# Thealexbarney/VGAudio

Measured on AMD Instinct MI355X. Metric: Msamples/s encoded (GC-ADPCM, 4096 ch) at 1/2/4/8 GPUs; % HBM roofline, higher is better.
Workload: dtype int32; 1 GPU; BASELINE configs[1]: 4096 mono channels x 48 kHz x 60 s GC-ADPCM coefficient search + encode per GPU; parallelism=units sharded x1, channels_per_gpu=4096, samples_per_channel=2880000, bit_exact_channels_checked=0

## Files before the change

include/vgaudio_hip_testing.h:

```cpp
#ifndef VGAUDIO_HIP_TESTING_H
#define VGAUDIO_HIP_TESTING_H

#ifdef __cplusplus
extern "C" {
#endif

int vga_testing_force_open_seams_this_thread(int mode);

int vga_testing_gc_encoder_layout_this_thread(int channels_per_wave);
int vga_testing_gc_coefs_variant_this_thread(int variant);
int vga_testing_gc_encoder_segments_this_thread(int segments);
int vga_testing_gc_encoder_persistent_this_thread(int mode);

int vga_testing_gc_plan_pieces(int cus, int groups, int frames, long long group_frames, int ragged, int *out5);

int vga_testing_gc_encode_stats(unsigned long long *out8, int reset);

void vga_testing_host_pipeline_this_thread(int feeders, int drainers, int chunk_units, int slot_bytes);

void vga_testing_host_pipeline_tail_this_thread(int tail_units);

int vga_testing_plan_buckets(const int *group, const int *length, int n, int max_units, long long max_volume, int longest_first,
                             int *order_out, int *chunk_begin_out, int *chunk_length_out, int *chunk_group_out, int max_chunks);
void vga_testing_buckets_order_this_thread(int order);
void vga_testing_host_transfer_this_thread(int mode);
void vga_testing_host_transfer_piece_bytes_this_thread(int bytes);
void vga_testing_host_compute_lanes_this_thread(int lanes);

enum {
    VGA_TESTING_STEP_CHUNK_COMPUTE = 1,
    VGA_TESTING_STEP_TRANSFER = 2,
    VGA_TESTING_STEP_HCA_STREAM_FRAMES = 3
};
void vga_testing_fail_step_this_thread(int kind, int nth);

int vga_testing_last_pipeline_stats(double *out, int n);

int vga_testing_hca_frames_per_group_this_thread(int frames);

int vga_testing_hca_device_info(const void *hca_info, void *out, int out_bytes);

int vga_testing_hca_decode_classes(const void *infos, int nstreams, int *class_out);
int vga_testing_hca_decode_v_stats(long long *out, int n);
int vga_testing_hca_ragged_stats(const void *ragged, long long *out, int n);

int vga_testing_adx_read_general_this_thread(int on);

int vga_testing_adx_last_path_this_thread(int *encode, int *decode);
int vga_testing_adx_ragged_stats(const void *ragged, long long *out, int n);
// ... 8 lines not shown
```

vgaudio_amd/_lib.py:

```python
import ctypes as C
import importlib.util
import os

_HERE = os.path.dirname(os.path.abspath(__file__))
SO_PATH = os.environ.get("VGAUDIO_HIP_LIBRARY") or os.path.join(_HERE, "libvgaudio_hip.so")

VGA_OK = 0
VGA_ERR_ARGUMENT = -1
VGA_ERR_OUT_OF_RANGE = -2
VGA_ERR_INVALID_DATA = -3
VGA_ERR_INVALID_OP = -4
VGA_ERR_DEVICE = -5

VGA_TESTING_STEP_CHUNK_COMPUTE = 1
VGA_TESTING_STEP_TRANSFER = 2
VGA_TESTING_STEP_HCA_STREAM_FRAMES = 3


class VgaError(RuntimeError):
    code = None


class ArgumentError(VgaError, ValueError):
    code = VGA_ERR_ARGUMENT
# ... 169 lines not shown
    "vga_gc_files_offsets": (ci, [vp, C.POINTER(ci), C.POINTER(i64), C.POINTER(i64)]),
    "vga_gc_files_ragged": (vp, [vp]),
    "vga_gcadpcm_build_channels_device_v": (ci, [vp, vp, vp, vp, vp, vp, vp, vp, C.c_size_t, vp]),
    "vga_dsp_write_device_v": (ci, [vp, vp, vp, vp, vp, vp, vp, vp]),
    "vga_dsp_read_device_v": (ci, [vp, vp, vp, vp, vp, vp, vp, vp]),
    "vga_gc_aligned_layout_for": (ci, [vp, ci, C.POINTER(ci), C.POINTER(i64), vp]),
    "vga_gc_aligned_create": (ci, [vp, ci, C.POINTER(vp)]),
    "vga_gc_aligned_destroy": (None, [vp]),
    "vga_gc_aligned_totals_of": (ci, [vp, vp]),
    "vga_gc_aligned_offsets": (ci, [vp, C.POINTER(ci), C.POINTER(i64)]),
    "vga_gc_aligned_ragged_in": (vp, [vp]),
    "vga_gc_aligned_ragged_out": (vp, [vp]),
    "vga_gcadpcm_align_channels_device_v": (ci, [vp, vp, vp, vp, vp, vp, vp, vp, vp, C.c_size_t, vp]),
    "vga_nw_files_layout_for": (ci, [vp, ci, vp, C.POINTER(ci), C.POINTER(i64), C.POINTER(i64), vp]),
    "vga_nw_files_create": (ci, [vp, ci, vp, C.POINTER(vp)]),
    "vga_nw_files_create_from_infos": (ci, [C.POINTER(vp), ci, C.POINTER(i64), C.POINTER(vp)]),
    "vga_nw_files_destroy": (None, [vp]),
    "vga_nw_files_totals_of": (ci, [vp, vp]),
    "vga_nw_files_offsets": (ci, [vp, C.POINTER(ci), C.POINTER(i64), C.POINTER(i64)]),
    "vga_nw_files_gc_files": (ci, [vp, vp]),
    "vga_nw_files_ragged": (vp, [vp]),
    "vga_nwstm_write_device_v": (ci, [vp, vp, vp, vp, vp, vp, vp, vp, vp]),
    "vga_nwstm_read_device_v": (ci, [vp, vp, vp, vp, vp, vp, vp, vp]),
    "vga_hca_decode_device_v": (ci, [vp, vp, vp, vp, C.c_size_t, vp, vp]),
    "vga_hca_encode_device_v": (ci, [vp, vp, vp, vp, vp]),
    "vga_hca_stream_create": (ci, [vp, vp, C.POINTER(vp)]),
    "vga_hca_stream_encode": (ci, [vp, vp, u8p, C.POINTER(ci)]),
    "vga_hca_stream_pending_frame_count": (ci, [vp]),
    "vga_hca_stream_get_pending_frame": (ci, [vp, u8p]),
    "vga_hca_stream_frames_processed": (ci, [vp]),
    "vga_hca_stream_frame_size": (ci, [vp]),
    "vga_hca_stream_destroy": (None, [vp]),
    "vga_testing_gc_encode_stats": (ci, [C.POINTER(C.c_ulonglong), ci]),
    "vga_testing_gc_plan_pieces": (ci, [ci, ci, ci, C.c_longlong, ci, C.POINTER(ci)]),
    "vga_set_devices": (ci, [vp, ci]),
    "vga_set_progress_callback": (ci, [vp, vp]),
    "vga_get_devices": (ci, [vp, ci]),
    "vga_testing_hca_frames_per_group_this_thread": (ci, [ci]),
    "vga_dsp_layout_for": (ci, [vp, ci, vp]),
    "vga_dsp_write": (ci, [u8pp, ci, i16p, i16p, i16p, i16p, ci, vp, u8p]),
    "vga_dsp_write_device": (ci, [vp, i64, ci, vp, vp, vp, vp, ci, vp, vp, vp]),
    "vga_nwstm_layout_for": (ci, [vp, ci, vp]),
    "vga_nwstm_write_device": (ci, [vp, ci, ci, vp, vp, i64, ci, vp, vp, vp, vp, vp, i64, ci, vp, i64, vp]),
    "vga_nwstm_write": (ci, [vp, ci, vp, u8pp, ci, i16p, i16p, i16p, i16p, i16pp, ci, u8p]),
    "vga_nwstm_parse": (ci, [u8p, C.c_size_t, vp]),
    "vga_nwstm_read_device": (ci, [vp, vp, i64, ci, vp, i64, vp]),
    "vga_nwstm_read": (ci, [u8p, C.c_size_t, vp, u8pp, i16pp]),
    "vga_pcm8_encode_device": (ci, [vp, i64, ci, ci, ci, vp, i64, vp]),
    "vga_pcm8_decode_device": (ci, [vp, i64, ci, ci, ci, vp, i64, vp]),
    "vga_nwstm_pcm_layout_for": (ci, [vp, ci, ci, vp]),
    "vga_nwstm_pcm_write_device": (ci, [vp, ci, ci, ci, vp, vp, ci, i64, vp, i64, vp]),
    "vga_nwstm_pcm_write": (ci, [vp, ci, ci, vp, vp, ci, u8p]),
    "vga_nwstm_pcm_parse": (ci, [u8p, C.c_size_t, vp]),
    "vga_nwstm_pcm_read_device": (ci, [vp, vp, i64, ci, vp, ci, i64, vp]),
    "vga_nwstm_pcm_read": (ci, [u8p, C.c_size_t, vp, vp, ci]),
    "vga_nwwav_parse": (ci, [u8p, C.c_size_t, vp]),
    "vga_nwwav_read": (ci, [u8p, C.c_size_t, vp, u8pp]),
    "vga_nwwav_bank_create": (ci, [vp, C.POINTER(i64), ci, C.POINTER(vp)]),
    "vga_nwwav_bank_destroy": (None, [vp]),
    "vga_nwwav_bank_channels": (ci, [vp]),
    "vga_nwwav_bank_codec_channels": (ci, [vp, ci]),
    "vga_nwwav_bank_rows": (ci, [vp, C.POINTER(ci), C.POINTER(ci), C.POINTER(ci), C.POINTER(ci), C.POINTER(i64)]),
    "vga_nwwav_bank_gc_sample_counts": (ci, [vp, C.POINTER(ci)]),
    "vga_nwwav_bank_gc_tables": (ci, [vp, i16p, i16p, i16p, i16p]),
    "vga_nwwav_bank_adpcm_bytes": (i64, [vp]),
    "vga_nwwav_bank_pcm16_samples": (i64, [vp]),
# ... 397 lines not shown
```

vgaudio_amd/csrc/common.hpp:

```cpp
#pragma once
#include <hip/hip_runtime.h>
#include <cstdarg>
#include <cstdint>
#include <cstdio>
#include <cstdlib>
#include <cstring>
#include <mutex>
#include <vector>

#include "../../include/vgaudio_hip.h"
#include "poison.hpp"

namespace vga {

void set_error(const char *fmt, ...);
bool take_error_pending();

#define VGA_HIP_TRY(expr)                                                              \
    do {                                                                               \
        hipError_t _e = (expr);                                                        \
        if (_e != hipSuccess) {                                                        \
            vga::set_error("%s failed: %s (%s:%d)", #expr, hipGetErrorString(_e),      \
                           __FILE__, __LINE__);                                        \
            return VGA_ERR_DEVICE;                                                     \
// ... 170 lines not shown
inline hipError_t allow_dynamic_lds(F *kernel, size_t bytes)
{
    return hipFuncSetAttribute(reinterpret_cast<const void *>(kernel), hipFuncAttributeMaxDynamicSharedMemorySize, (int)bytes);
}

struct Stream {
    hipStream_t s = nullptr;
    ~Stream() { if (s) (void)hipStreamDestroy(s); }
    hipError_t create() { return hipStreamCreateWithFlags(&s, hipStreamNonBlocking); }
};

inline int64_t round_up(int64_t v, int64_t m) { return (v + m - 1) / m * m; }

__device__ __forceinline__ void lds_barrier()
{
#if defined(__HIP_DEVICE_COMPILE__)
    asm volatile("s_waitcnt lgkmcnt(0)\n\ts_barrier" ::: "memory");
#endif
}

int require_device();

inline int device_cu_count()
{
    int device = 0, cus = 256;
    if (hipGetDevice(&device) == hipSuccess) (void)hipDeviceGetAttribute(&cus, hipDeviceAttributeMultiprocessorCount, device);
    return cus > 0 ? cus : 256;
}

int force_open_seams();

int encoder_layout();
int coefs_kernel_variant();
int encoder_segments_override();
int encoder_persistent_mode();
int hca_frames_per_group_override();
void note_adx_encode_path(int path);
void note_adx_decode_path(int path);

__host__ __device__ inline bool seam_forced_open(int mode, int channel, int seam)
{
    return mode == 1 || mode == 3 || (mode == 2 && channel % 3 == 0 && seam % 2 == 0);
}

}
```

vgaudio_amd/csrc/gc_encode_core.hpp:

```cpp
#pragma once
#include <cstdint>

#if defined(__HIPCC__)
#define VGA_HD __host__ __device__ __forceinline__
#else
#define VGA_HD inline
#endif

#if defined(__HIP_DEVICE_COMPILE__)
#define VGA_MUL24(a, b) __mul24((a), (b))
#define VGA_OPAQUE(v) asm("" : "+v"(v))
#define VGA_OPAQUE_S(v) asm("" : "+s"(v))
static __device__ __forceinline__ uint32_t vga_square24(int e)
{
    uint32_t r;
    asm("v_mul_i32_i24 %0, %1, %1" : "=v"(r) : "v"(e));
    return r;
}
#else
#define VGA_MUL24(a, b) ((a) * (b))
#define VGA_OPAQUE(v) ((void)0)
#define VGA_OPAQUE_S(v) ((void)0)
#endif

// ... 596 lines not shown
}

VGA_HD PassOut resume_passes_core(const int (&x)[16], const int (&in2048p)[14], int c0, int c1, int scale_power,
                                  int &final_sp)
{
    PassOut r;
    bool at_max;
    do {
        scale_power++;
        at_max = scale_power >= 12;
        r = pass_fast_core(x, pack16(x[0], x[1]), in2048p, c0, c1, scale_power);
        if (!r.exact) r = pass_literal(x, c0, c1, scale_power);
        scale_power = apply_bumps(scale_power, r.max_overflow);
    } while (scale_power < 12 && r.max_overflow > 1 && !at_max);
    final_sp = scale_power;
    return r;
}

VGA_HD PassOut resume_passes(const int (&x)[16], int c0, int c1, int scale_power, int &final_sp)
{
    PassOut r;
    bool at_max;
    do {
        scale_power++;
        at_max = scale_power >= 12;
        r = pass_fast(x, c0, c1, scale_power);
        if (!r.exact) r = pass_literal(x, c0, c1, scale_power);
        scale_power = apply_bumps(scale_power, r.max_overflow);
    } while (scale_power < 12 && r.max_overflow > 1 && !at_max);
    final_sp = scale_power;
    return r;
}

}
}
```

vgaudio_amd/csrc/gc_encode_kernel.hip:

```cpp
#include "common.hpp"
#include "gc_encode_core.hpp"
#include "gcadpcm_kernels.hpp"
#include "seams.hpp"
#include "gc_plan8.hpp"

#include <cstdio>
#include <cstdlib>

namespace vga {
namespace gc {

constexpr int DPP_QUAD_XOR1 = 0xB1;
constexpr int DPP_QUAD_XOR2 = 0x4E;
constexpr int DPP_ROW_HALF_MIRROR = 0x141;
constexpr int DPP_ROW_MIRROR = 0x140;

template <int CTRL>
__device__ __forceinline__ int dpp(int v)
{
    return __builtin_amdgcn_update_dpp(0, v, CTRL, 0xF, 0xF, true);
}

__device__ __forceinline__ unsigned umin32(unsigned a, unsigned b) { return a < b ? a : b; }

template <class Op>
__device__ __forceinline__ unsigned row16_reduce(unsigned v, Op op)
{
    v = op(v, (unsigned)dpp<DPP_QUAD_XOR1>((int)v));
    v = op(v, (unsigned)dpp<DPP_QUAD_XOR2>((int)v));
    v = op(v, (unsigned)dpp<DPP_ROW_HALF_MIRROR>((int)v));
    v = op(v, (unsigned)dpp<DPP_ROW_MIRROR>((int)v));
    return v;
}


#ifdef VGA_DEBUG_TIMESTAMPS
__device__ unsigned long long g_vga_enc_ts[1 << 16];
extern "C" int vga_debug_encode_timestamps(unsigned long long *out, int n)
{
    return (int)hipMemcpyFromSymbol(out, HIP_SYMBOL(g_vga_enc_ts), (size_t)n * sizeof(unsigned long long));
}
#endif
__device__ unsigned long long g_vga_gc_stats[8];
extern "C" int vga_testing_gc_encode_stats(unsigned long long *out8, int reset)
{
    if (hipDeviceSynchronize() != hipSuccess) return -1;
    if (out8 && hipMemcpyFromSymbol(out8, HIP_SYMBOL(g_vga_gc_stats), 8 * sizeof(unsigned long long)) != hipSuccess) return -1;
#ifdef VGA_GC_STATS
    if (out8) out8[7] = 1;
#else
    if (out8) out8[7] = 0;
#endif
    if (reset) {
        const unsigned long long zero[8] = {0, 0, 0, 0, 0, 0, 0, 0};
        if (hipMemcpyToSymbol(HIP_SYMBOL(g_vga_gc_stats), zero, sizeof zero) != hipSuccess) return -1;
    }
    return 0;
}
constexpr int SW = 2;
constexpr int ENC_THREADS = 64 * (SW + 1);
#ifndef VGA_GC_ENCODER_PRIO
#define VGA_GC_ENCODER_PRIO 3
#endif
#ifndef VGA_GC_HELPER_PRIO
#define VGA_GC_HELPER_PRIO 0
#endif
#ifndef VGA_GC_PERSISTENT_WAVES_PER_EU
#define VGA_GC_PERSISTENT_WAVES_PER_EU 3, 3
#endif
template <int CPW, bool SELF = false>
struct Lay {
    static_assert(!SELF || CPW == 8, "the self-served shape is the (channel, predictor) layout");
    static constexpr int EW = SELF ? 1 : SW;
    static constexpr int CS = CPW * EW;
    static constexpr int TF = 64 / CS;
    static constexpr int THREADS = SELF ? 64 : ENC_THREADS;
    static constexpr int BUFS = SELF ? 1 : 2;
};
template <int CS, int TF>
struct GcTileT {
    struct Slot {
        uint32_t xw[8];
        int in2048p[16];
        uint32_t pre[8];
        int4 out[4];
    };
    struct Group { Slot f[TF]; uint32_t pad[4]; };
    Group g[CS];
// ... 766 lines not shown
        {                                                                              \
            const unsigned olo = (unsigned)dpp<CTRL>((int)(uint32_t)key);              \
            const unsigned ohi = (unsigned)dpp<CTRL>((int)(uint32_t)(key >> 32));      \
            const uint64_t okey = ((uint64_t)ohi << 32) | olo;                         \
            key = okey < key ? okey : key;                                             \
        }
        VGA_MIN64_STAGE(DPP_QUAD_XOR1)
        VGA_MIN64_STAGE(DPP_QUAD_XOR2)
        VGA_MIN64_STAGE(DPP_ROW_HALF_MIRROR)
        if (LPC == 16) VGA_MIN64_STAGE(DPP_ROW_MIRROR)
#undef VGA_MIN64_STAGE
        const bool won = act && fin && lidx == (int)(key & 15u);
        unsigned pay = won ? r.hist_pair : 0u;
        pay |= (unsigned)dpp<DPP_QUAD_XOR1>((int)pay);
        pay |= (unsigned)dpp<DPP_QUAD_XOR2>((int)pay);
        pay |= (unsigned)dpp<DPP_ROW_HALF_MIRROR>((int)pay);
        if (LPC == 16) pay |= (unsigned)dpp<DPP_ROW_MIRROR>((int)pay);
        if (won) {
            uint32_t d0, d1;
            pack_frame(r.q, pr, final_sp, d0, d1);
            *reinterpret_cast<uint2 *>(dst + f * 8) = make_uint2(d0, d1);
        }
        if (act) {
            h0 = (int)(int16_t)(pay & 0xFFFF);
            h1 = (int)pay >> 16;
            if (h0 == g2 && h1 == g1 && !seam_forced_open(force_open, ch, k)) open = false;
        }
#pragma unroll
        for (int i = 0; i < 7; i++) w[i] = wn[i];
        old = oldn;
    }
}

template <int LPC>
__device__ __forceinline__ void encode_tail_frame(const int16_t *__restrict__ src, uint8_t *__restrict__ dst, int c0, int c1,
                                                  bool coef_ok, int pr, int total_samples, int h0, int h1, bool act)
{
    const int full_frames = total_samples / 14, tail = total_samples - full_frames * 14;
    int x[16], mp[14];
    x[0] = h0;
    x[1] = h1;
    const uint32_t hpk = pack16(h0, h1);
#pragma unroll
    for (int i = 0; i < 14; i++) x[2 + i] = i < tail ? (int)src[(int64_t)full_frames * 14 + i] : 0;
#pragma unroll
    for (int i = 0; i < 14; i++) mp[i] = x[2 + i] * 2048 + 1024;
    int s1;
    {
        int dmax = 0, dmin = 0;
        prescan_range(x, c0, c1, 0, 14, dmax, dmin);
        s1 = first_scale_power_from_range(dmax, dmin);
        if (s1 == -100) s1 = first_scale_power_from_md(prescan_sequential(x, c0, c1));
    }
    const int sp_a = imin(s1, 12), sp_b = imin(s1 + 1, 12);
    uint32_t w[7];
    pack_row(x, w);
    const PassOut rb = pass_fast_core(w, hpk, mp, c0, c1, sp_b);
    const PassOut ra = pass_fast_core(w, hpk, mp, c0, c1, sp_a);
    const bool cap_a = sp_a >= 12, cap_b = sp_b >= 12;
    const bool rare = !coef_ok || (unsigned)ra.max_overflow > (cap_a ? 2u : 248u) || (unsigned)rb.max_overflow > (cap_b ? 2u : 248u);
    const int eff_a = cap_a ? 0 : ra.max_overflow, eff_b = cap_b ? 0 : rb.max_overflow;
    const bool fin_a = eff_a < 2;
    const bool resume = !fin_a && eff_b >= 2;
    PassOut r;
#pragma unroll
    for (int i = 0; i < 14; i++) r.q[i] = fin_a ? ra.q[i] : rb.q[i];
    r.total = fin_a ? ra.total : rb.total;
    int final_sp = fin_a ? sp_a : sp_b;
    if (rare || resume) {
        const PassOut rc = resume_passes(x, c0, c1, rare ? s1 - 1 : s1 + 1, final_sp);
#pragma unroll
        for (int i = 0; i < 14; i++) r.q[i] = rc.q[i];
        r.total = rc.total;
    }
    const bool in_it = act && (LPC == 8 || (threadIdx.x & 1) == 0);
    uint64_t key = in_it ? ((r.total << 3) | (uint64_t)pr) : ~0ull;
#define VGA_MIN64_STAGE(CTRL)                                                          \
    {                                                                                  \
        const unsigned olo = (unsigned)dpp<CTRL>((int)(uint32_t)key);                  \
        const unsigned ohi = (unsigned)dpp<CTRL>((int)(uint32_t)(key >> 32));          \
        const uint64_t okey = ((uint64_t)ohi << 32) | olo;                             \
        key = okey < key ? okey : key;                                                 \
    }
    VGA_MIN64_STAGE(DPP_QUAD_XOR1)
    VGA_MIN64_STAGE(DPP_QUAD_XOR2)
    VGA_MIN64_STAGE(DPP_ROW_HALF_MIRROR)
    if (LPC == 16) VGA_MIN64_STAGE(DPP_ROW_MIRROR)
#undef VGA_MIN64_STAGE
    if (in_it && pr == (int)(key & 7u)) {
        uint32_t d0, d1;
        pack_frame(r.q, pr, final_sp, d0, d1);
        const int nibbles = tail + 2;
        store_frame_bytes(dst + (int64_t)full_frames * 8, d0, d1, nibbles / 2 + (nibbles & 1));
    }
}

template <int LPC>
__device__ __forceinline__ void seam_piece(
    const int slot_raw, const int k, const int lane,
    const int16_t *__restrict__ pcm, int64_t pcm_pitch, int nch, int total_samples, const Pieces seg,
    const int16_t *__restrict__ coefs, uint8_t *adpcm, int64_t adpcm_pitch,
    const int16_t *seg_state, int *first_open, int *seam_flag, int *seam_end, int force_open, const Ragged &rg)
{
    const int pr = LPC == 16 ? (lane >> 1) & 7 : lane & 7;
    const bool lead = (lane & (LPC - 1)) == 0;
    const int64_t f0 = seg.first(k);
    const int slot = slot_raw < nch ? slot_raw : nch - 1;
    const int ch = rg.order ? rg.order[slot] : slot;
    if (rg.order) total_samples = rg.length[ch];
    const bool valid = slot_raw < nch && f0 * 14 < total_samples;
    const int16_t *src = pcm + (rg.order ? rg.pcm_off[ch] : (int64_t)ch * pcm_pitch);
    uint8_t *dst = adpcm + (rg.order ? rg.adpcm_off[ch] : (int64_t)ch * adpcm_pitch);
    const int16_t *cf = coefs + ch * 16;
    const int c0 = cf[2 * pr], c1 = cf[2 * pr + 1];
    const bool coef_ok = (c0 < 0 ? -c0 : c0) + (c1 < 0 ? -c1 : c1) <= 32767;
    int h0 = valid ? seg_state[((int64_t)(k - 1) * nch + ch) * 2] : 0;
    int h1 = valid ? seg_state[((int64_t)(k - 1) * nch + ch) * 2 + 1] : 0;
    const int g2 = valid ? src[f0 * 14 - 2] : 0, g1 = valid ? src[f0 * 14 - 1] : 0;
    bool open = valid;
    int frames_run = 0;
    seam_run<LPC>(src, dst, c0, c1, coef_ok, pr, ch, k, f0, total_samples, seg.frames(k), seg.frames(k), force_open, h0, h1, g2, g1, open, frames_run);
    if (valid && lead) {
        atomicAdd(&g_vga_gc_stats[open ? 1 : 0], 1ull);
        atomicAdd(&g_vga_gc_stats[2], (unsigned long long)frames_run);
        seam_flag[(int64_t)(k - 1) * nch + ch] = open ? 1 : 0;
        if (open) {
            seam_end[(int64_t)(k - 1) * nch + ch] = (int)(((unsigned)h1 << 16) | ((unsigned)h0 & 0xFFFFu));
            atomicMin(&first_open[ch], k);
        }
    }
}

template <int LPC>
__global__ __launch_bounds__(64) void gc_encode_seam_kernel(
    const int16_t *__restrict__ pcm, int64_t pcm_pitch, int nch, int total_samples, const Pieces seg,
    const int16_t *__restrict__ coefs, uint8_t *__restrict__ adpcm, int64_t adpcm_pitch,
    const int16_t *__restrict__ seg_state, int *__restrict__ first_open, int *__restrict__ seam_flag,
    int *__restrict__ seam_end, int force_open, const Ragged rg)
{
    seam_piece<LPC>(blockIdx.x * (64 / LPC) + (threadIdx.x / LPC), blockIdx.y + 1, threadIdx.x, pcm, pcm_pitch, nch, total_samples, seg, coefs, adpcm,
               adpcm_pitch, seg_state, first_open, seam_flag, seam_end, force_open, rg);
}

template <int CPW, bool RAGGED>
__global__ __launch_bounds__(ENC_THREADS) __attribute__((amdgpu_waves_per_eu(VGA_GC_PERSISTENT_WAVES_PER_EU))) void gc_encode_persistent_kernel(
    const int16_t *__restrict__ pcm, int64_t pcm_pitch, int nch, int total_samples, const Pieces seg,
    const int16_t *__restrict__ coefs, const int16_t *__restrict__ hist1,
    const int16_t *__restrict__ hist2, uint8_t *adpcm, int64_t adpcm_pitch, int16_t *seg_state,
    const Ragged rg, int groups, int segments, int *__restrict__ queue, int *__restrict__ seam_count, int *first_open,
    int *seam_flag, int *seam_end, int force_open)
{
    static_assert(CPW == 8, "the seams inside the persistent kernel use the (channel, predictor) layout");
    constexpr int CS = Lay<CPW>::CS;
    __shared__ int s_item;
// ... 13 lines not shown
#endif
            return;
        }
        int g = item % groups, y = item / groups;
        if (RAGGED && rg.items) {
            const uint32_t v = rg.items[item];
            g = (int)(v & 0xFFFFFu);
            y = (int)(v >> 20);
        }
        gc_encode_piece<false, CPW, RAGGED>(g, y, pcm, pcm_pitch, nch, total_samples, seg, coefs, hist1, hist2, adpcm, adpcm_pitch,
                                            seg_state, (const int *)nullptr, rg);
        if (segments <= 1) continue;
        __threadfence();
        __syncthreads();
        if (threadIdx.x == 0) {
            const int total_wg = RAGGED ? rg.length[rg.order[g * CS]] : total_samples;
            auto exists = [&](int piece) { return piece < segments && seg.first(piece) * 14 < total_wg; };
            int at_start = 0, at_end = 0;
            if (exists(y)) {
                if (y >= 1 && atomicAdd(&seam_count[(int64_t)(y - 1) * groups + g], 1) == 1) at_start = y;
                if (exists(y + 1) && atomicAdd(&seam_count[(int64_t)y * groups + g], 1) == 1) at_end = y + 1;
            }
            s_seam[0] = at_start;
            s_seam[1] = at_end;
        }
        __syncthreads();
        const int seam_a = s_seam[0], seam_b = s_seam[1];
        if ((seam_a | seam_b) != 0) {
            __threadfence();
            const int wave = threadIdx.x >> 6, lane = threadIdx.x & 63;
            if (wave < SW) {
                const int slot = g * CS + wave * CPW + (lane >> 3);
                if (seam_a)
                    seam_piece<8>(slot, seam_a, lane, pcm, pcm_pitch, nch, total_samples, seg, coefs, adpcm, adpcm_pitch, seg_state,
                               first_open, seam_flag, seam_end, force_open, rg);
                if (seam_b)
                    seam_piece<8>(slot, seam_b, lane, pcm, pcm_pitch, nch, total_samples, seg, coefs, adpcm, adpcm_pitch, seg_state,
                               first_open, seam_flag, seam_end, force_open, rg);
            }
        }
    }
}

template <bool RAGGED>
__global__ __launch_bounds__(64) __attribute__((amdgpu_waves_per_eu(3, 3))) void gc_encode_self_served_kernel(
    const int16_t *__restrict__ pcm, int64_t pcm_pitch, int nch, int total_samples, const Pieces seg,
    const int16_t *__restrict__ coefs, const int16_t *__restrict__ hist1,
    const int16_t *__restrict__ hist2, uint8_t *adpcm, int64_t adpcm_pitch, int16_t *seg_state,
    const Ragged rg, int groups, int items, int segments, int *__restrict__ queue, int *__restrict__ seam_count, int *first_open,
    int *seam_flag, int *seam_end, int force_open)
{
    constexpr int CS = PLAN8_SLOTS;
    static_assert(Lay<8, true>::CS == CS && Lay<8, true>::THREADS == 64, "one wave, eight channel slots");
    const int lane = threadIdx.x;
    const uint32_t *host_items = RAGGED ? rg.items : nullptr;
#ifdef VGA_DEBUG_TIMESTAMPS
    if (lane == 0) g_vga_enc_ts[2 * (blockIdx.x & 32767)] = wall_clock64();
#endif
    for (;;) {
        int item = 0;
        if (lane == 0) item = atomicAdd(queue, 1);
        item = __builtin_amdgcn_readfirstlane(item);
        if (item >= items) {
#ifdef VGA_DEBUG_TIMESTAMPS
            if (lane == 0) g_vga_enc_ts[2 * (blockIdx.x & 32767) + 1] = wall_clock64();
#endif
            return;
        }
        int g, y;
        if (!plan8_item(item, groups, nch, host_items, g, y)) continue;
        gc_encode_piece<false, 8, RAGGED, true>(g, y, pcm, pcm_pitch, nch, total_samples, seg, coefs, hist1, hist2, adpcm, adpcm_pitch,
                                                seg_state, (const int *)nullptr, rg);
        if (segments <= 1) continue;
        __threadfence();
        int at_start = 0, at_end = 0;
        if (lane == 0) {
            const int total_wg = RAGGED ? rg.length[rg.order[g * CS]] : total_samples;
            auto exists = [&](int piece) { return piece < segments && seg.first(piece) * 14 < total_wg; };
            if (exists(y)) {
                if (y >= 1 && atomicAdd(&seam_count[(int64_t)(y - 1) * groups + g], 1) == 1) at_start = y;
                if (exists(y + 1) && atomicAdd(&seam_count[(int64_t)y * groups + g], 1) == 1) at_end = y + 1;
            }
        }
        const int seam_a = __builtin_amdgcn_readfirstlane(at_start), seam_b = __builtin_amdgcn_readfirstlane(at_end);
        if ((seam_a | seam_b) != 0) {
            __threadfence();
            const int slot = g * CS + (lane >> 3);
            if (seam_a)
                seam_piece<8>(slot, seam_a, lane, pcm, pcm_pitch, nch, total_samples, seg, coefs, adpcm, adpcm_pitch, seg_state,
                           first_open, seam_flag, seam_end, force_open, rg);
            if (seam_b)
                seam_piece<8>(slot, seam_b, lane, pcm, pcm_pitch, nch, total_samples, seg, coefs, adpcm, adpcm_pitch, seg_state,
                           first_open, seam_flag, seam_end, force_open, rg);
        }
    }
}

template <int LPC>
__global__ __launch_bounds__(64) void gc_encode_chain_kernel(
    const int16_t *__restrict__ pcm, int64_t pcm_pitch, int nch, int total_samples, const Pieces seg, int segments,
    const int16_t *__restrict__ coefs, uint8_t *__restrict__ adpcm, int64_t adpcm_pitch,
    int16_t *__restrict__ seg_state, int *__restrict__ first_open, const int *__restrict__ seam_flag,
    const int *__restrict__ seam_end, int force_open, const Ragged rg)
{
    const int lane = threadIdx.x;
    const int pr = LPC == 16 ? (lane >> 1) & 7 : lane & 7;
    const bool lead = (lane & (LPC - 1)) == 0;
    const int slot_raw = blockIdx.x * (64 / LPC) + lane / LPC;
    const bool live = slot_raw < nch;
    const int slot = live ? slot_raw : nch - 1;
    const int ch = rg.order ? rg.order[slot] : slot;
    if (rg.order) total_samples = rg.length[ch];
    const int mine = live ? first_open[ch] : SEAM_NONE;
    int kmin = mine;
#pragma unroll
    for (int o = LPC; o < 64; o <<= 1) kmin = imin(kmin, __shfl_xor(kmin, o));
    if (kmin >= segments) return;
    if (live && lead && mine < segments) atomicAdd(&g_vga_gc_stats[5], 1ull);
    int frames_run = 0;
    const int16_t *src = pcm + (rg.order ? rg.pcm_off[ch] : (int64_t)ch * pcm_pitch);
    uint8_t *dst = adpcm + (rg.order ? rg.adpcm_off[ch] : (int64_t)ch * adpcm_pitch);
    const int16_t *cf = coefs + ch * 16;
    const int c0 = cf[2 * pr], c1 = cf[2 * pr + 1];
    const bool coef_ok = (c0 < 0 ? -c0 : c0) + (c1 < 0 ? -c1 : c1) <= 32767;
    bool have = false;
    int v0 = 0, v1 = 0;
// ... 159 lines not shown
    }
    const bool self = want_self && persistent;
    const Plan8 p8 = self ? plan_groups_of_eight(cus, nch, segments, RAGGED && rg.items ? rg.n_items : -1) : Plan8{};
    const int seam_groups = self ? p8.groups : groups;
    AsyncBuf scratch;
    int16_t *seg_state = nullptr;
    int *first_open = nullptr, *seam_flag = nullptr, *seam_end = nullptr, *queue = nullptr, *seam_count = nullptr;
    if (segments > 1 || persistent) {
        const size_t state_bytes = segments > 1 ? (size_t)round_up((int64_t)segments * nch * 2 * (int64_t)sizeof(int16_t), 16) : 0;
        const size_t open_bytes = (size_t)round_up((int64_t)nch * (int64_t)sizeof(int), 16);
        const size_t count_bytes = persistent && segments > 1 ? (size_t)round_up((int64_t)(segments - 1) * seam_groups * (int64_t)sizeof(int), 16) : 0;
        const size_t need = 3 * state_bytes + open_bytes + 16 + count_bytes;
        unsigned char *base = static_cast<unsigned char *>(d_scratch);
        if (!base || scratch_bytes < need) {
            VGA_HIP_TRY(scratch.alloc(need, stream));
            base = scratch.as<unsigned char>();
        }
        seam_flag = reinterpret_cast<int *>(base + state_bytes);
        seam_end = reinterpret_cast<int *>(base + 2 * state_bytes);
        first_open = reinterpret_cast<int *>(base + 3 * state_bytes);
        queue = reinterpret_cast<int *>(base + 3 * state_bytes + open_bytes);
        if (segments > 1) {
            seg_state = reinterpret_cast<int16_t *>(base);
            VGA_HIP_TRY(fill_no_open_seams(first_open, nch, stream));
        } else
            seg_state = nullptr;
        seam_count = queue + 4;
        if (persistent) VGA_HIP_TRY(hipMemsetAsync(queue, 0, 16 + count_bytes, stream));
    }
    if (self) {
        if constexpr (CPW == 8)
            hipLaunchKernelGGL((gc_encode_self_served_kernel<RAGGED>), dim3(p8.wgs), dim3(Lay<8, true>::THREADS), 0, stream, d_pcm, pcm_pitch,
                               nch, sample_count, seg, d_coefs, d_hist1, d_hist2, d_adpcm, adpcm_pitch, seg_state, rg, p8.groups, p8.items,
                               segments, queue, seam_count, first_open, seam_flag, seam_end, force_open_seams());
    } else if (persistent) {
        const int items = RAGGED && rg.items ? rg.n_items : groups * segments;
        const int wgs = imin(items, cus * persistent_wgs_per_cu());
        if constexpr (CPW == 8)
            hipLaunchKernelGGL((gc_encode_persistent_kernel<CPW, RAGGED>), dim3(wgs), dim3(ENC_THREADS), 0, stream, d_pcm, pcm_pitch, nch,
                               sample_count, seg, d_coefs, d_hist1, d_hist2, d_adpcm, adpcm_pitch, seg_state, rg, groups, segments, queue,
                               seam_count, first_open, seam_flag, seam_end, force_open_seams());
    } else
        hipLaunchKernelGGL((gc_encode_kernel<false, CPW, RAGGED>), dim3(groups, segments), dim3(ENC_THREADS), 0, stream, d_pcm, pcm_pitch, nch,
                           sample_count, seg, d_coefs, d_hist1, d_hist2, d_adpcm, adpcm_pitch, seg_state,
                           (const int *)nullptr, rg);
    VGA_HIP_TRY(hipGetLastError());
    if (segments > 1) {
        if (!persistent) {
#ifdef VGA_GC_SEAM16_ALWAYS
            const bool wide = CPW == 4;
#else
            const bool wide = CPW == 4 && nch > 64;
#endif
            if (wide)
                hipLaunchKernelGGL(gc_encode_seam_kernel<16>, dim3((nch + 3) / 4, segments - 1), dim3(64), 0, stream, d_pcm, pcm_pitch, nch,
                                   sample_count, seg, d_coefs, d_adpcm, adpcm_pitch, seg_state, first_open, seam_flag, seam_end,
                                   force_open_seams(), rg);
            else
                hipLaunchKernelGGL(gc_encode_seam_kernel<8>, dim3((nch + 7) / 8, segments - 1), dim3(64), 0, stream, d_pcm, pcm_pitch, nch,
                                   sample_count, seg, d_coefs, d_adpcm, adpcm_pitch, seg_state, first_open, seam_flag, seam_end,
                                   force_open_seams(), rg);
            VGA_HIP_TRY(hipGetLastError());
        }
#ifdef VGA_GC_SEAM16_ALWAYS
        if (CPW == 4)
#else
        if (CPW == 4 && nch > 64)
// ... 38 lines not shown
```

vgaudio_amd/csrc/host_batch.hpp:

```cpp
#pragma once
#include <algorithm>
#include <atomic>
#include <cstdlib>
#include <memory>
#include <mutex>
#include "common.hpp"
#include "host_pipeline.hpp"
#include "../../include/vgaudio_hip_testing.h"

namespace vga {

struct PipeOverride {
    int feeders = 0, drainers = 0, chunk_units = 0, slot_bytes = 0, tail_units = 0;
    int buckets_order = 0;
    int transfer = 0;
    int piece_bytes = 0;
    int compute_lanes = 0;
};
struct FailStep {
    int kind = 0, nth = 0, seen = 0;
};
constexpr const char *kRefusedStep = "step refused by vga_testing_fail_step_this_thread";
int launch_transfer(const pipe::Job::TransferPiece *pieces, int n, hipStream_t stream);
int device_cu_count();

struct ThreadSettings {
    int force_open_seams = 0;
    int encoder_layout = 0;
    int coefs_variant = 0;
    int encoder_segments = 0;
    int encoder_persistent = 0;
    int hca_frames_per_group = 0;
    PipeOverride pipe;
    FailStep fail;
};
ThreadSettings &thread_settings();
inline PipeOverride &pipe_override() { return thread_settings().pipe; }
inline bool refuse_step(int kind)
{
    FailStep &f = thread_settings().fail;
    return f.kind == kind && ++f.seen == f.nth;
}
struct PipeReport { pipe::Stats stats; double t_alloc = 0, t_entry = 0; };
PipeReport &pipe_report();
int hardware_queues_requested();
inline int planned_compute_lanes(int own_choice)
{
    const int hook = pipe_override().compute_lanes;
    return std::max(1, std::min(hook > 0 ? hook : own_choice, pipe::kMaxComputeLanes));
}

std::vector<int> batch_devices();

struct ProgressCallback { void (*fn)(void *user, int64_t done, int64_t total) = nullptr; void *user = nullptr; };
ProgressCallback progress_callback();
struct ProgressSink {
    ProgressCallback cb;
    int64_t total = 0, done = 0;
    std::mutex m;
    void add(int64_t units)
    {
        std::lock_guard<std::mutex> g(m);
        done += units;
        cb.fn(cb.user, done, total);
// ... 312 lines not shown
```

vgaudio_amd/csrc/runtime.hip:

```cpp
#include "common.hpp"
#include "host_batch.hpp"
#include "../../include/vgaudio_hip_testing.h"

namespace vga {

static thread_local char g_err[512] = "";
static thread_local bool g_err_pending = false;

void set_error(const char *fmt, ...)
{
    va_list ap;
    va_start(ap, fmt);
    vsnprintf(g_err, sizeof g_err, fmt, ap);
    va_end(ap);
    g_err_pending = true;
}

bool take_error_pending()
{
    const bool was = g_err_pending;
    g_err_pending = false;
    return was;
}

int require_device()
{
    g_err_pending = false;
    int n = 0;
    hipError_t e = hipGetDeviceCount(&n);
    if (e != hipSuccess || n <= 0) {
        set_error("no HIP device available (%s); libvgaudio_hip has no CPU fallback",
                  e == hipSuccess ? "device count 0" : hipGetErrorString(e));
        return VGA_ERR_DEVICE;
    }
    return VGA_OK;
}

static thread_local ThreadSettings g_settings;
ThreadSettings &thread_settings() { return g_settings; }
int force_open_seams() { return g_settings.force_open_seams; }
int encoder_layout() { return g_settings.encoder_layout; }
int coefs_kernel_variant() { return g_settings.coefs_variant; }
int encoder_segments_override() { return g_settings.encoder_segments; }
int encoder_persistent_mode() { return g_settings.encoder_persistent; }
int hca_frames_per_group_override() { return g_settings.hca_frames_per_group; }
static thread_local int g_adx_encode_path = 0, g_adx_decode_path = 0;
void note_adx_encode_path(int path) { g_adx_encode_path = path; }
void note_adx_decode_path(int path) { g_adx_decode_path = path; }

static int g_queues_seen_by_runtime = 4;
__attribute__((constructor)) static void read_hardware_queues()
{
    if (const char *host = std::getenv("GPU_MAX_HW_QUEUES"))
        g_queues_seen_by_runtime = std::atoi(host);
}
int hardware_queues_requested() { return g_queues_seen_by_runtime; }

static std::mutex g_devices_mutex;
static std::vector<int> g_devices;
std::vector<int> batch_devices()
{
    std::lock_guard<std::mutex> g(g_devices_mutex);
    return g_devices;
}

static thread_local PipeReport g_pipe_report;
PipeReport &pipe_report() { return g_pipe_report; }
static thread_local ProgressCallback g_progress_callback;
ProgressCallback progress_callback() { return g_progress_callback; }
static thread_local ProgressSink *g_progress_sink = nullptr;
ProgressSink *&current_progress_sink() { return g_progress_sink; }

}

using namespace vga;

// ... 45 lines not shown
    return (int)g_devices.size();
}

int vga_set_progress_callback(vga_progress_fn fn, void *user)
{
    g_progress_callback.fn = fn;
    g_progress_callback.user = fn ? user : nullptr;
    return VGA_OK;
}

int vga_testing_force_open_seams_this_thread(int mode)
{
    const int old = g_settings.force_open_seams;
    g_settings.force_open_seams = mode;
    return old;
}
int vga_testing_gc_encoder_layout_this_thread(int channels_per_wave)
{
    const int old = g_settings.encoder_layout;
    if (channels_per_wave == 0 || channels_per_wave == 1 || channels_per_wave == 4 || channels_per_wave == 8)
        g_settings.encoder_layout = channels_per_wave;
    return old;
}
int vga_testing_gc_coefs_variant_this_thread(int variant)
{
    const int old = g_settings.coefs_variant;
    if (variant >= 0 && variant <= 3) g_settings.coefs_variant = variant;
    return old;
}
int vga_testing_gc_encoder_segments_this_thread(int segments)
{
    const int old = g_settings.encoder_segments;
    g_settings.encoder_segments = segments > 0 ? segments : 0;
    return old;
}
int vga_testing_gc_encoder_persistent_this_thread(int mode)
{
    const int old = g_settings.encoder_persistent;
    g_settings.encoder_persistent = mode >= 0 && mode <= 2 ? mode : 0;
    return old;
}
int vga_testing_hca_frames_per_group_this_thread(int frames)
{
    const int old = g_settings.hca_frames_per_group;
    g_settings.hca_frames_per_group = frames > 0 ? frames : 0;
    return old;
}
int vga_testing_adx_last_path_this_thread(int *encode, int *decode)
{
    if (encode) *encode = g_adx_encode_path;
    if (decode) *decode = g_adx_decode_path;
    return 0;
}
void vga_testing_host_pipeline_this_thread(int feeders, int drainers, int chunk_units, int slot_bytes)
{
    PipeOverride &o = g_settings.pipe;
    o.feeders = feeders;
    o.drainers = drainers;
    o.chunk_units = chunk_units;
    o.slot_bytes = slot_bytes;
}
void vga_testing_host_pipeline_tail_this_thread(int tail_units) { g_settings.pipe.tail_units = tail_units > 0 ? tail_units : 0; }
void vga_testing_buckets_order_this_thread(int order) { g_settings.pipe.buckets_order = order == 1 || order == 2 ? order : 0; }
void vga_testing_host_transfer_this_thread(int mode) { g_settings.pipe.transfer = mode == 1 || mode == 2 ? mode : 0; }
void vga_testing_host_transfer_piece_bytes_this_thread(int bytes) { g_settings.pipe.piece_bytes = bytes > 0 ? bytes : 0; }
void vga_testing_fail_step_this_thread(int kind, int nth)
// ... 40 lines not shown
```

Baseline: 85770 Msamples/s.

## Add lean seam-repair path for GC-ADPCM self-served encoder

Adds a lean seam-run routine for the self-served encoder. It replays the previously encoded frame's nibbles to track the guessed history, and it uses a cheaper first-scale/final-pass path with wave-uniform cold fallbacks and DPP min reductions to pick the winning predictor. The lean path is enabled by default through a mode bit packed into the force_open argument, unless seam mode 1 is selected. It also turns the two seam calls into a non-unrolled loop to cut code size and register pressure, and adds optional seam statistics. The risk is extra divergence on cold or saturated frames and added code complexity in a rarely dominant seam phase.

```diff
diff --git a/include/vgaudio_hip_testing.h b/include/vgaudio_hip_testing.h
--- a/include/vgaudio_hip_testing.h
+++ b/include/vgaudio_hip_testing.h
@@ -15,6 +15,10 @@
 int vga_testing_gc_plan_pieces(int cus, int groups, int frames, long long group_frames, int ragged, int *out5);
 
 int vga_testing_gc_encode_stats(unsigned long long *out8, int reset);
+
+int vga_testing_gc_seam_stats(unsigned long long *out8, int reset);
+
+int vga_testing_gc_seam_mode_this_thread(int mode);
 
 void vga_testing_host_pipeline_this_thread(int feeders, int drainers, int chunk_units, int slot_bytes);
 
diff --git a/vgaudio_amd/_lib.py b/vgaudio_amd/_lib.py
--- a/vgaudio_amd/_lib.py
+++ b/vgaudio_amd/_lib.py
@@ -225,6 +225,8 @@
     "vga_hca_stream_frame_size": (ci, [vp]),
     "vga_hca_stream_destroy": (None, [vp]),
     "vga_testing_gc_encode_stats": (ci, [C.POINTER(C.c_ulonglong), ci]),
+    "vga_testing_gc_seam_stats": (ci, [C.POINTER(C.c_ulonglong), ci]),
+    "vga_testing_gc_seam_mode_this_thread": (ci, [ci]),
     "vga_testing_gc_plan_pieces": (ci, [ci, ci, ci, C.c_longlong, ci, C.POINTER(ci)]),
     "vga_set_devices": (ci, [vp, ci]),
     "vga_set_progress_callback": (ci, [vp, vp]),
diff --git a/vgaudio_amd/csrc/common.hpp b/vgaudio_amd/csrc/common.hpp
--- a/vgaudio_amd/csrc/common.hpp
+++ b/vgaudio_amd/csrc/common.hpp
@@ -226,6 +226,7 @@
 
 int encoder_layout();
 int coefs_kernel_variant();
+int gc_seam_mode();
 int encoder_segments_override();
 int encoder_persistent_mode();
 int hca_frames_per_group_override();
diff --git a/vgaudio_amd/csrc/gc_encode_core.hpp b/vgaudio_amd/csrc/gc_encode_core.hpp
--- a/vgaudio_amd/csrc/gc_encode_core.hpp
+++ b/vgaudio_amd/csrc/gc_encode_core.hpp
@@ -652,5 +652,97 @@
     return r;
 }
 
-}
-}
+VGA_HD uint32_t alignbit16(uint32_t hi, uint32_t lo)
+{
+#if defined(__HIP_DEVICE_COMPILE__)
+    return __builtin_amdgcn_alignbit(hi, lo, 16);
+#else
+    return (hi << 16) | (lo >> 16);
+#endif
+}
+VGA_HD void seam_lean_rows(const uint32_t (&w)[7], int (&a2048)[14], int (&in_b)[14])
+{
+#if defined(__HIP_DEVICE_COMPILE__)
+#pragma unroll
+#endif
+    for (int i = 0; i < 7; i++) {
+        a2048[2 * i] = pair_lo(w[i]) * 2048;
+        a2048[2 * i + 1] = pair_hi(w[i]) * 2048;
+    }
+#if defined(__HIP_DEVICE_COMPILE__)
+#pragma unroll
+#endif
+    for (int i = 0; i < 14; i++) in_b[i] = a2048[i] + (1024 + PASS_B_OFF);
+}
+VGA_HD int seam_lean_first_scale(const uint32_t (&w)[7], const int (&a2048)[14], const int (&in_b)[14], uint32_t hist, uint32_t cpk,
+                                 uint32_t ncpk, int &P0_b, int &sum, int &pos)
+{
+    uint32_t pair[12];
+    int a12[12];
+#if defined(__HIP_DEVICE_COMPILE__)
+#pragma unroll
+#endif
+    for (int k = 0; k < 12; k++) {
+        pair[k] = (k & 1) ? alignbit16(w[(k + 1) / 2], w[(k - 1) / 2]) : w[k / 2];
+        a12[k] = a2048[k + 2];
+    }
+    const uint32_t pre = prescan_numer_word(pair, a12, ncpk);
+    P0_b = predicted_b(hist, cpk);
+    const int d0 = head_distance_numer_b(in_b[0], P0_b);
+    const int d1 = head_distance_numer_b(in_b[1], predicted_b(alignbit16(w[0], hist), cpk));
+    const int dmax = imax(imax(pair_lo(pre), d0), d1);
+    const int dmin = imin(imin(pair_hi(pre), d0), d1);
+    return first_scale_power_nt(dmax, dmin, sum, pos);
+}
+struct SeamLane {
+    int q[14];
+    uint32_t hist_pair;
+    int final_sp;
+    uint64_t total;
+    bool sum_exact;
+};
+VGA_HD void seam_lean_cold(const uint32_t (&w)[7], uint32_t hist, int c0, int c1, int s1, int sp_a, int sp_b, int ov_a, int ov_2,
+                           SeamLane &o)
+{
+    const FrameFlags ff = frame_flags(sp_a, sp_b, ov_a, ov_2, true);
+    if (ff.generic || ff.resume) {
+        int x[16];
+        unpack_row(w, hist, x);
+        const PassOut rc = resume_passes(x, c0, c1, ff.generic ? s1 - 1 : s1 + 1, o.final_sp);
+#if defined(__HIP_DEVICE_COMPILE__)
+#pragma unroll
+#endif
+        for (int i = 0; i < 14; i++) o.q[i] = rc.q[i];
+        o.hist_pair = rc.hist_pair;
+        o.total = rc.total;
+        o.sum_exact = true;
+    }
+}
+VGA_HD uint64_t seam_lean_exact_total(const uint32_t (&w)[7], uint32_t hist, int c0, int c1, const SeamLane &o)
+{
+    if (!needs_exact_sum(o.total, o.sum_exact)) return o.total;
+    int row[14];
+#if defined(__HIP_DEVICE_COMPILE__)
+#pragma unroll
+#endif
+    for (int i = 0; i < 7; i++) {
+        row[2 * i] = pair_lo(w[i]) * 2048 + 1024;
+        row[2 * i + 1] = pair_hi(w[i]) * 2048 + 1024;
+    }
+    return pass_fast_core_wide(w, hist, row, c0, c1, o.final_sp).total;
+}
+VGA_HD uint32_t seam_replay_step(uint32_t g, uint32_t kpk, int k, int nibble)
+{
+    const int acc = (int)((uint32_t)nibble << k) + 1024;
+    return sat_pack16(pair_hi(g), dot2_i16(g, kpk, acc) >> 11);
+}
+VGA_HD int seam_frame_nibble(uint32_t d0, uint32_t d1, int s)
+{
+    const int byte = 1 + (s >> 1);
+    const uint32_t word = byte < 4 ? d0 : d1;
+    const int off = 8 * (byte & 3) + ((s & 1) ? 0 : 4);
+    return (int)(word << (28 - off)) >> 28;
+}
+
+}
+}
diff --git a/vgaudio_amd/csrc/gc_encode_kernel.hip b/vgaudio_amd/csrc/gc_encode_kernel.hip
--- a/vgaudio_amd/csrc/gc_encode_kernel.hip
+++ b/vgaudio_amd/csrc/gc_encode_kernel.hip
@@ -54,6 +54,23 @@
     if (reset) {
         const unsigned long long zero[8] = {0, 0, 0, 0, 0, 0, 0, 0};
         if (hipMemcpyToSymbol(HIP_SYMBOL(g_vga_gc_stats), zero, sizeof zero) != hipSuccess) return -1;
+    }
+    return 0;
+}
+__device__ unsigned long long g_vga_gc_seam_stats[8];
+[[maybe_unused]] constexpr int SEAM_STATS_FIRST_RUN = 64;
+extern "C" int vga_testing_gc_seam_stats(unsigned long long *out8, int reset)
+{
+    if (hipDeviceSynchronize() != hipSuccess) return -1;
+    if (out8 && hipMemcpyFromSymbol(out8, HIP_SYMBOL(g_vga_gc_seam_stats), 8 * sizeof(unsigned long long)) != hipSuccess) return -1;
+#ifdef VGA_GC_STATS
+    if (out8) out8[7] = 1;
+#else
+    if (out8) out8[7] = 0;
+#endif
+    if (reset) {
+        const unsigned long long zero[8] = {0, 0, 0, 0, 0, 0, 0, 0};
+        if (hipMemcpyToSymbol(HIP_SYMBOL(g_vga_gc_seam_stats), zero, sizeof zero) != hipSuccess) return -1;
     }
     return 0;
 }
@@ -886,6 +903,110 @@
     }
 }
 
+__device__ __forceinline__ void seam_run_lean(const int16_t *__restrict__ src, uint8_t *__restrict__ dst, int c0, int c1,
+                                              int pr, int ch, int k, int64_t f0, int total_samples, int piece_frames, int max_frames, int force_open,
+                                              int &h0, int &h1, int g2, int g1, bool &open, int &frames_run)
+{
+    const int full_frames = total_samples / 14;
+    const int64_t f_end = imin((int)imin((int)(f0 + piece_frames), (int)(f0 + max_frames)), full_frames);
+    const int64_t f_last = full_frames > 0 ? full_frames - 1 : 0;
+    auto fetch = [&](int64_t f, uint32_t (&w)[7], uint2 &old) {
+        const int64_t fc = f < f_last ? f : f_last;
+        const uint32_t *p32 = reinterpret_cast<const uint32_t *>(src + fc * 14);
+#pragma unroll
+        for (int i = 0; i < 7; i++) w[i] = p32[i];
+        old = *reinterpret_cast<const uint2 *>(dst + fc * 8);
+    };
+    const uint32_t cpk = pack16(c1, c0), ncpk = pack16(-c1, -c0);
+    uint32_t hpk = pack16(h0, h1), gpk = pack16(g2, g1);
+    uint32_t w[7], wn[7];
+    uint2 old, oldn;
+    fetch(f0, w, old);
+    for (int64_t f = f0; ; f++) {
+        const bool in_range = f < f_end;
+        if (!__any(open && in_range)) break;
+        const bool act = open && in_range;
+        frames_run += act ? 1 : 0;
+        fetch(f + 1, wn, oldn);
+        {
+            const int ps = (int)(old.x & 0xFFu);
+            const int kk = 11 + (ps & 0xF);
+            const uint32_t kpk = (uint32_t)__shfl((int)cpk, (ps >> 4) & 7, 8);
+#pragma unroll
+            for (int s2 = 0; s2 < 14; s2++) gpk = seam_replay_step(gpk, kpk, kk, seam_frame_nibble(old.x, old.y, s2));
+        }
+        int a2048[14], mp[14];
+        seam_lean_rows(w, a2048, mp);
+        int P0, sum, pos;
+        int s1 = seam_lean_first_scale(w, a2048, mp, hpk, cpk, ncpk, P0, sum, pos);
+        if (__builtin_expect(__builtin_amdgcn_ballot_w64(sum == 0) != 0, 0)) {
+            if (sum == 0 && first_scale_tie(pos)) {
+                int x[16];
+                unpack_row(w, hpk, x);
+                s1 = first_scale_power_from_md(prescan_sequential(x, c0, c1));
+            }
+        }
+        const int sp_a = imin(s1, 12), sp_b = imin(s1 + 1, 12);
+        PassOutB r;
+        int ov_a, sp2;
+        r = final_pass_pair<false>(w, hpk, mp, c0, c1, sp_a, sp_b, P0, ov_a, sp2);
+        const int ov_2 = r.max_overflow;
+        const bool cold = act && frame_goes_cold(sp_a, sp_b, ov_a, ov_2, true).cold;
+        SeamLane o;
+#pragma unroll
+        for (int i = 0; i < 14; i++) o.q[i] = r.q2[i];
+        o.hist_pair = r.hist_pair;
+        o.final_sp = sp2;
+        o.total = error_sum_pairs(w, r.pairs);
+        o.sum_exact = false;
+        if (__builtin_expect(__builtin_amdgcn_ballot_w64(cold) != 0, 0)) {
+            if (cold) seam_lean_cold(w, hpk, c0, c1, s1, sp_a, sp_b, ov_a, ov_2, o);
+        }
+        constexpr unsigned SAT = (1u << 28) - 1;
+        const unsigned tot = umin32((unsigned)(o.total >> 32) ? SAT : (unsigned)o.total, SAT);
+        unsigned key = act ? ((tot << 3) | (unsigned)pr) : 0xFFFFFFFFu;
+        key = umin32(key, (unsigned)dpp<DPP_QUAD_XOR1>((int)key));
+        key = umin32(key, (unsigned)dpp<DPP_QUAD_XOR2>((int)key));
+        key = umin32(key, (unsigned)dpp<DPP_ROW_HALF_MIRROR>((int)key));
+        int winner = (int)(key & 7u);
+        if (__builtin_expect(__any(act && (key >> 3) >= SAT), 0)) {
+            const uint64_t total = seam_lean_exact_total(w, hpk, c0, c1, o);
+            uint64_t key64 = act ? ((total << 3) | (uint64_t)pr) : ~0ull;
+#define VGA_MIN64_STAGE(CTRL)                                                          \
+            {                                                                          \
+                const unsigned olo = (unsigned)dpp<CTRL>((int)(uint32_t)key64);        \
+                const unsigned ohi = (unsigned)dpp<CTRL>((int)(uint32_t)(key64 >> 32)); \
+                const uint64_t okey = ((uint64_t)ohi << 32) | olo;                     \
+                key64 = okey < key64 ? okey : key64;                                   \
+            }
+            VGA_MIN64_STAGE(DPP_QUAD_XOR1)
+            VGA_MIN64_STAGE(DPP_QUAD_XOR2)
+            VGA_MIN64_STAGE(DPP_ROW_HALF_MIRROR)
+#undef VGA_MIN64_STAGE
+            if ((key >> 3) >= SAT) winner = (int)(key64 & 7u);
+        }
+        const bool won = act && pr == winner;
+        unsigned pay = won ? o.hist_pair : 0u;
+        pay |= (unsigned)dpp<DPP_QUAD_XOR1>((int)pay);
+        pay |= (unsigned)dpp<DPP_QUAD_XOR2>((int)pay);
+        pay |= (unsigned)dpp<DPP_ROW_HALF_MIRROR>((int)pay);
+        if (won) {
+            uint32_t d0, d1;
+            pack_frame_mod16(o.q, pr, o.final_sp, d0, d1);
+            *reinterpret_cast<uint2 *>(dst + f * 8) = make_uint2(d0, d1);
+        }
+        if (act) {
+            hpk = pay;
+            if (hpk == gpk && !seam_forced_open(force_open, ch, k)) open = false;
+        }
+#pragma unroll
+        for (int i = 0; i < 7; i++) w[i] = wn[i];
+        old = oldn;
+    }
+    h0 = pair_lo(hpk);
+    h1 = pair_hi(hpk);
+}
+
 template <int LPC>
 __device__ __forceinline__ void encode_tail_frame(const int16_t *__restrict__ src, uint8_t *__restrict__ dst, int c0, int c1,
                                                   bool coef_ok, int pr, int total_samples, int h0, int h1, bool act)
@@ -949,13 +1070,15 @@
     }
 }
 
-template <int LPC>
+constexpr int SEAM_LEAN_BIT = 256;
+template <int LPC, bool QUEUED = false, bool LEAN = false>
 __device__ __forceinline__ void seam_piece(
     const int slot_raw, const int k, const int lane,
     const int16_t *__restrict__ pcm, int64_t pcm_pitch, int nch, int total_samples, const Pieces seg,
     const int16_t *__restrict__ coefs, uint8_t *adpcm, int64_t adpcm_pitch,
-    const int16_t *seg_state, int *first_open, int *seam_flag, int *seam_end, int force_open, const Ragged &rg)
-{
+    const int16_t *seg_state, int *first_open, int *seam_flag, int *seam_end, int force_open_and_mode, const Ragged &rg)
+{
+    const int force_open = LEAN ? force_open_and_mode & (SEAM_LEAN_BIT - 1) : force_open_and_mode;
     const int pr = LPC == 16 ? (lane >> 1) & 7 : lane & 7;
     const bool lead = (lane & (LPC - 1)) == 0;
     const int64_t f0 = seg.first(k);
@@ -973,7 +1096,31 @@
     const int g2 = valid ? src[f0 * 14 - 2] : 0, g1 = valid ? src[f0 * 14 - 1] : 0;
     bool open = valid;
     int frames_run = 0;
-    seam_run<LPC>(src, dst, c0, c1, coef_ok, pr, ch, k, f0, total_samples, seg.frames(k), seg.frames(k), force_open, h0, h1, g2, g1, open, frames_run);
+#ifdef VGA_GC_ABLATE_SEAMS
+    if (QUEUED) open = false;
+    else
+#endif
+    if (LEAN && LPC == 8 && (force_open_and_mode & SEAM_LEAN_BIT) != 0 && __builtin_amdgcn_ballot_w64(!pass_b_coef_ok(c0, c1)) == 0)
+        seam_run_lean(src, dst, c0, c1, pr, ch, k, f0, total_samples, seg.frames(k), seg.frames(k), force_open, h0, h1, g2, g1, open, frames_run);
+    else
+        seam_run<LPC>(src, dst, c0, c1, coef_ok, pr, ch, k, f0, total_samples, seg.frames(k), seg.frames(k), force_open, h0, h1, g2, g1, open, frames_run);
+#ifdef VGA_GC_STATS
+    if (QUEUED) {
+        int longest = frames_run;
+        for (int m = 32; m >= 1; m >>= 1) longest = imax(longest, __shfl_xor(longest, m, 64));
+        if (lane == 0) {
+            atomicAdd(&g_vga_gc_seam_stats[0], (unsigned long long)longest);
+            atomicAdd(&g_vga_gc_seam_stats[4], 1ull);
+        }
+        if (valid && lead) {
+            atomicAdd(&g_vga_gc_seam_stats[1], (unsigned long long)frames_run);
+            if (frames_run > SEAM_STATS_FIRST_RUN) {
+                atomicAdd(&g_vga_gc_seam_stats[5], 1ull);
+                atomicAdd(&g_vga_gc_seam_stats[6], (unsigned long long)(frames_run - SEAM_STATS_FIRST_RUN));
+            }
+        }
+    }
+#endif
     if (valid && lead) {
         atomicAdd(&g_vga_gc_stats[open ? 1 : 0], 1ull);
         atomicAdd(&g_vga_gc_stats[2], (unsigned long long)frames_run);
@@ -1053,10 +1200,10 @@
             if (wave < SW) {
                 const int slot = g * CS + wave * CPW + (lane >> 3);
                 if (seam_a)
-                    seam_piece<8>(slot, seam_a, lane, pcm, pcm_pitch, nch, total_samples, seg, coefs, adpcm, adpcm_pitch, seg_state,
+                    seam_piece<8, true>(slot, seam_a, lane, pcm, pcm_pitch, nch, total_samples, seg, coefs, adpcm, adpcm_pitch, seg_state,
                                first_open, seam_flag, seam_end, force_open, rg);
                 if (seam_b)
-                    seam_piece<8>(slot, seam_b, lane, pcm, pcm_pitch, nch, total_samples, seg, coefs, adpcm, adpcm_pitch, seg_state,
+                    seam_piece<8, true>(slot, seam_b, lane, pcm, pcm_pitch, nch, total_samples, seg, coefs, adpcm, adpcm_pitch, seg_state,
                                first_open, seam_flag, seam_end, force_open, rg);
             }
         }
@@ -1106,13 +1253,16 @@
         const int seam_a = __builtin_amdgcn_readfirstlane(at_start), seam_b = __builtin_amdgcn_readfirstlane(at_end);
         if ((seam_a | seam_b) != 0) {
             __threadfence();
-            const int slot = g * CS + (lane >> 3);
-            if (seam_a)
-                seam_piece<8>(slot, seam_a, lane, pcm, pcm_pitch, nch, total_samples, seg, coefs, adpcm, adpcm_pitch, seg_state,
-                           first_open, seam_flag, seam_end, force_open, rg);
-            if (seam_b)
-                seam_piece<8>(slot, seam_b, lane, pcm, pcm_pitch, nch, total_samples, seg, coefs, adpcm, adpcm_pitch, seg_state,
-                           first_open, seam_flag, seam_end, force_open, rg);
+            int lane_s = lane;
+            asm volatile("" : "+v"(lane_s));
+            const int slot = g * CS + (lane_s >> 3);
+#pragma clang loop unroll(disable)
+            for (int end = 0; end < 2; end++) {
+                const int seam = end == 0 ? seam_a : seam_b;
+                if (seam)
+                    seam_piece<8, true, true>(slot, seam, lane_s, pcm, pcm_pitch, nch, total_samples, seg, coefs, adpcm, adpcm_pitch, seg_state,
+                               first_open, seam_flag, seam_end, force_open, rg);
+            }
         }
     }
 }
@@ -1338,7 +1488,8 @@
         if constexpr (CPW == 8)
             hipLaunchKernelGGL((gc_encode_self_served_kernel<RAGGED>), dim3(p8.wgs), dim3(Lay<8, true>::THREADS), 0, stream, d_pcm, pcm_pitch,
                                nch, sample_count, seg, d_coefs, d_hist1, d_hist2, d_adpcm, adpcm_pitch, seg_state, rg, p8.groups, p8.items,
-                               segments, queue, seam_count, first_open, seam_flag, seam_end, force_open_seams());
+                               segments, queue, seam_count, first_open, seam_flag, seam_end,
+                               force_open_seams() | (gc_seam_mode() != 1 ? SEAM_LEAN_BIT : 0));
     } else if (persistent) {
         const int items = RAGGED && rg.items ? rg.n_items : groups * segments;
         const int wgs = imin(items, cus * persistent_wgs_per_cu());
diff --git a/vgaudio_amd/csrc/host_batch.hpp b/vgaudio_amd/csrc/host_batch.hpp
--- a/vgaudio_amd/csrc/host_batch.hpp
+++ b/vgaudio_amd/csrc/host_batch.hpp
@@ -30,6 +30,7 @@
     int coefs_variant = 0;
     int encoder_segments = 0;
     int encoder_persistent = 0;
+    int gc_seam_mode = 0;
     int hca_frames_per_group = 0;
     PipeOverride pipe;
     FailStep fail;
diff --git a/vgaudio_amd/csrc/runtime.hip b/vgaudio_amd/csrc/runtime.hip
--- a/vgaudio_amd/csrc/runtime.hip
+++ b/vgaudio_amd/csrc/runtime.hip
@@ -42,6 +42,7 @@
 int encoder_layout() { return g_settings.encoder_layout; }
 int coefs_kernel_variant() { return g_settings.coefs_variant; }
 int encoder_segments_override() { return g_settings.encoder_segments; }
+int gc_seam_mode() { return g_settings.gc_seam_mode; }
 int encoder_persistent_mode() { return g_settings.encoder_persistent; }
 int hca_frames_per_group_override() { return g_settings.hca_frames_per_group; }
 static thread_local int g_adx_encode_path = 0, g_adx_decode_path = 0;
@@ -153,6 +154,12 @@
 {
     const int old = g_settings.encoder_segments;
     g_settings.encoder_segments = segments > 0 ? segments : 0;
+    return old;
+}
+int vga_testing_gc_seam_mode_this_thread(int mode)
+{
+    const int old = g_settings.gc_seam_mode;
+    if (mode >= 0 && mode <= 3) g_settings.gc_seam_mode = mode;
     return old;
 }
 int vga_testing_gc_encoder_persistent_this_thread(int mode)
```

Result: no change. 86540 Msamples/s, median of 3 (+0.9%).
